# yang-0201/MAF-YOLO

Measured on AMD Instinct MI355X. Metric: images/sec MAF-YOLO-n 640x640 bs=32 infer (Model.forward + non_max_suppression), higher is better.
Workload: dtype f16

## Files before the change

maf-yolo_amd/csrc/conv1dw.hip:

```cpp
#include "maf_common.h"

namespace {

struct C1dArgs {
    const half_t* x; half_t* out;
    const unsigned char* par;
    int B, H, W, Cin, Cmid, S1, nMB, x_stride, x_coff, out_stride, out_coff;
    int tilesX, tilesY, nwg, rec;
};

typedef half_t half4v_t __attribute__((ext_vector_type(4)));

template <int K>
struct C1dCfg {
    static constexpr int P = K / 2, PARTS = K > 5 ? 2 : 1;
    static constexpr int RH = 16 + K - 1, RWC = (16 + K - 1 + 3) & ~3, NHP = RH * RWC, NPT = (NHP + 15) / 16;
    static constexpr int RWP = 24;
    static constexpr int PSB = ((RH * RWP * 2 - 8 + 255) / 256) * 256 + 8;
    static constexpr int PS = PSB / 2;
    static constexpr int NTOE = 8 * K * PARTS * 16;
};

template <int K>
__global__ __launch_bounds__(256) void conv1dw_kernel(const C1dArgs a) {
    typedef C1dCfg<K> Cf;
    constexpr int P = Cf::P, PARTS = Cf::PARTS, RWC = Cf::RWC, NHP = Cf::NHP, NPT = Cf::NPT, RWP = Cf::RWP, PS = Cf::PS;
    extern __shared__ __attribute__((aligned(16))) unsigned char smem_raw[];
    half_t* T1 = reinterpret_cast<half_t*>(smem_raw);
    unsigned char* rec = smem_raw + 32 * Cf::PSB;
    const int OFF_B1 = 2 * a.S1 * 1024, OFF_TOE = OFF_B1 + 128, OFF_BD = OFF_TOE + Cf::NTOE * 16;

    const int tid = threadIdx.x, wave = tid >> 6, lane = tid & 63, g = lane >> 4, p = lane & 15;
    const int lid = maf_xcd_contiguous_id(a.nwg);
    const int mb = lid % a.nMB;
    int tt = lid / a.nMB;
    const int tx = tt % a.tilesX; tt /= a.tilesX;
    const int ty = tt % a.tilesY;
    const int b = tt / a.tilesY;
    const int y0 = ty * 16, x0 = tx * 16;
    const half_t* xin = a.x + (size_t)b * a.H * a.W * a.x_stride + a.x_coff;

    {
        const unsigned char* src = a.par + (size_t)mb * a.rec;
        const int nvec = a.rec >> 4;
        for (int v0 = wave * 64; v0 < nvec; v0 += 256)
            if (v0 + lane < nvec)
                __builtin_amdgcn_global_load_lds((const void __attribute__((address_space(1)))*)(src + (size_t)(v0 + lane) * 16),
                                                 (void __attribute__((address_space(3)))*)(rec + v0 * 16), 16, 0, 0);
    }
    __syncthreads();

    {
        const bool interior = y0 - P >= 0 && x0 - P >= 0 && y0 - P + Cf::RH <= a.H && x0 - P + RWC <= a.W;
        const half8_t* w1l = reinterpret_cast<const half8_t*>(rec) + lane;
        const float b1v0 = reinterpret_cast<const float*>(rec + OFF_B1)[p], b1v1 = reinterpret_cast<const float*>(rec + OFF_B1)[16 + p];
        for (int t = wave; t < NPT; t += 4) {
            const int m = t * 16 + p;
            const int hrp = m / RWC, hcp = m - hrp * RWC;
            const int iy = min(max(y0 - P + hrp, 0), a.H - 1), ix = min(max(x0 - P + hcp, 0), a.W - 1);
            const half_t* px = xin + (size_t)(iy * a.W + ix) * a.x_stride;
            f32x4_t acc1[2] = {(f32x4_t)0.f, (f32x4_t)0.f};
            for (int ks0 = 0; ks0 < a.S1; ks0 += 4) {
                half8_t af[4];
#pragma unroll
                for (int u = 0; u < 4; ++u) {
                    int c = (ks0 + u) * 32 + g * 8;
                    c = c < a.Cin ? c : 0;
                    af[u] = *reinterpret_cast<const half8_t*>(px + c);
                }
#pragma unroll
                for (int u = 0; u < 4; ++u)
                    if (ks0 + u < a.S1) {
                        acc1[0] = __builtin_amdgcn_mfma_f32_16x16x32_f16(af[u], w1l[(0 * a.S1 + ks0 + u) * 64], acc1[0], 0, 0, 0);
                        acc1[1] = __builtin_amdgcn_mfma_f32_16x16x32_f16(af[u], w1l[(1 * a.S1 + ks0 + u) * 64], acc1[1], 0, 0, 0);
                    }
            }
            const int m0 = t * 16 + g * 4;
            const int hr = m0 / RWC, hc0 = m0 - hr * RWC;
            uint32_t mlo = 0xffffffffu, mhi = 0xffffffffu;
            if (!interior) {
                const int iy2 = y0 - P + hr, ixb = x0 - P + hc0;
                const bool rowok = (unsigned)iy2 < (unsigned)a.H;
                const uint32_t k0 = (rowok && (unsigned)(ixb + 0) < (unsigned)a.W) ? 0x0000ffffu : 0u, k1 = (rowok && (unsigned)(ixb + 1) < (unsigned)a.W) ? 0xffff0000u : 0u;
                const uint32_t k2 = (rowok && (unsigned)(ixb + 2) < (unsigned)a.W) ? 0x0000ffffu : 0u, k3 = (rowok && (unsigned)(ixb + 3) < (unsigned)a.W) ? 0xffff0000u : 0u;
                mlo = k0 | k1; mhi = k2 | k3;
            }
            half_t* dst = T1 + (size_t)p * PS + hr * RWP + hc0;
#pragma unroll
            for (int ct = 0; ct < 2; ++ct) {
                const float bv = ct ? b1v1 : b1v0;
                const half2_t h01 = {(half_t)maf_act<MAF_ACT_SILU>(acc1[ct][0] + bv), (half_t)maf_act<MAF_ACT_SILU>(acc1[ct][1] + bv)};
                const half2_t h23 = {(half_t)maf_act<MAF_ACT_SILU>(acc1[ct][2] + bv), (half_t)maf_act<MAF_ACT_SILU>(acc1[ct][3] + bv)};
                const u32x2_t w = {__builtin_bit_cast(uint32_t, h01) & mlo, __builtin_bit_cast(uint32_t, h23) & mhi};
                if (m0 < NHP) *reinterpret_cast<u32x2_t*>(dst + (size_t)(16 * ct) * PS) = w;
            }
        }
    }
    __syncthreads();

    const bool toe_active = (p >> 2) == g;
    const int q4 = wave * 4;
    int hi_off = 4;
    asm volatile("" : "+v"(hi_off));
    f32x4_t dacc[8];
#pragma unroll
    for (int s = 0; s < 8; ++s) dacc[s] = (f32x4_t)0.f;
    const half8_t* tl = reinterpret_cast<const half8_t*>(rec + OFF_TOE) + p;
    const half_t* t1l = T1 + (size_t)g * PS + p * RWP + q4;
    const half_t* t1h = t1l + hi_off;
#pragma unroll 1
    for (int ky = 0; ky < K; ++ky) {
#pragma unroll
        for (int part = 0; part < PARTS; ++part) {
#pragma unroll
            for (int s = 0; s < 8; ++s) {
                half8_t av = (half8_t)(half_t)0;
                if (toe_active) av = tl[((s * K + ky) * PARTS + part) * 16];
                const int o = s * 4 * PS + ky * RWP + part * 4;
                const half4v_t lo = *reinterpret_cast<const half4v_t*>(t1l + o), hi = *reinterpret_cast<const half4v_t*>(t1h + o);
                const half8_t bv = {lo[0], lo[1], lo[2], lo[3], hi[0], hi[1], hi[2], hi[3]};
                dacc[s] = __builtin_amdgcn_mfma_f32_16x16x32_f16(av, bv, dacc[s], 0, 0, 0);
            }
        }
    }
    const int c0 = mb * 32 + g * 8;
    if (c0 >= a.Cmid) return;
    const f32x4_t bd0 = reinterpret_cast<const f32x4_t*>(rec + OFF_BD)[g * 2], bd1 = reinterpret_cast<const f32x4_t*>(rec + OFF_BD)[g * 2 + 1];
    const float bs[8] = {bd0[0], bd0[1], bd0[2], bd0[3], bd1[0], bd1[1], bd1[2], bd1[3]};
    const int oy = y0 + p;
    if (oy >= a.H) return;
    half_t* orow = a.out + ((size_t)b * a.H + oy) * a.W * a.out_stride + a.out_coff + c0;
#pragma unroll
    for (int r = 0; r < 4; ++r) {
        const int ox = x0 + q4 + r;
        if (ox >= a.W) continue;
        half8_t o;
#pragma unroll
        for (int s = 0; s < 8; ++s) o[s] = (half_t)maf_act<MAF_ACT_SILU>(dacc[s][r] + bs[s]);
        *reinterpret_cast<half8_t*>(orow + (size_t)ox * a.out_stride) = o;
    }
}

template <int K>
int launch_k(const C1dArgs& a, hipStream_t s) {
    const size_t lds = (size_t)32 * C1dCfg<K>::PSB + (size_t)a.rec;
    MAF_REQUIRE(lds <= 160 * 1024, "conv1dw: tile + record do not fit LDS");
    static bool attr = false;
    if (!attr) {
        int rc = maf_check_hip(hipFuncSetAttribute(reinterpret_cast<const void*>(&conv1dw_kernel<K>), hipFuncAttributeMaxDynamicSharedMemorySize, 160 * 1024), "hipFuncSetAttribute(conv1dw)");
        if (rc) return rc;
        attr = true;
    }
    hipLaunchKernelGGL((conv1dw_kernel<K>), dim3(a.nwg), dim3(256), lds, s, a);
    return maf_check_hip(hipGetLastError(), "conv1dw launch");
}

}

extern "C" int64_t maf_conv1dw_record_bytes(int32_t k, int32_t Cin) {
    const int parts = k > 5 ? 2 : 1, s1 = (Cin + 31) / 32;
    return (int64_t)2 * s1 * 1024 + 128 + (int64_t)8 * k * parts * 16 * 16 + 128;
}

int maf_launch_conv1dw(const maf_op_t* op, hipStream_t s) {
    MAF_REQUIRE(op->dtype == MAF_F16, "conv1dw: fp16 only");
    const maf_src_t& sr = op->src[0];
    MAF_REQUIRE(op->nsrc == 1 && sr.mode == MAF_SRC_DIRECT && sr.ptr && op->out && op->w, "conv1dw: one direct source, w = block records");
    MAF_REQUIRE(op->Cin % 8 == 0 && op->Cout % 8 == 0 && op->Cin <= 512, "conv1dw: Cin, Cmid multiples of 8, Cin <= 512");
    MAF_REQUIRE(sr.stride % 8 == 0 && sr.coff % 8 == 0 && op->out_stride % 8 == 0 && op->out_coff % 8 == 0, "conv1dw: stride/offset alignment");
    MAF_REQUIRE(op->act == MAF_ACT_SILU, "conv1dw: SiLU after both stages (common.py:905-909)");
    C1dArgs a;
    a.x = static_cast<const half_t*>(sr.ptr); a.out = static_cast<half_t*>(op->out);
    a.par = static_cast<const unsigned char*>(op->w);
    a.B = op->B; a.H = op->H; a.W = op->W; a.Cin = op->Cin; a.Cmid = op->Cout; a.S1 = (op->Cin + 31) / 32; a.nMB = (op->Cout + 31) / 32;
    a.x_stride = sr.stride; a.x_coff = sr.coff; a.out_stride = op->out_stride; a.out_coff = op->out_coff;
    a.tilesX = maf_cdiv(a.W, 16); a.tilesY = maf_cdiv(a.H, 16);
    a.nwg = a.B * a.tilesX * a.tilesY * a.nMB;
    a.rec = (int)maf_conv1dw_record_bytes(op->ksize, op->Cin);
    switch (op->ksize) {
        case 3: return launch_k<3>(a, s);
        case 5: return launch_k<5>(a, s);
        case 7: return launch_k<7>(a, s);
        case 9: return launch_k<9>(a, s);
        default: maf_set_error("conv1dw: k must be 3, 5, 7 or 9"); return MAF_E_UNSUPPORTED;
    }
}
```

maf-yolo_amd/plan_report.py:

```python
from . import lib, pack

_ESIZE = {lib.F16: 2, lib.F32: 4}


def kernel_name(plan, idx):
    o = plan.ops[idx]
    T = "_Float16" if o.dtype == lib.F16 else "float"
    if o.kind in (lib.OP_CONV1X1, lib.OP_CONV3X3S2):
        if o.kind == lib.OP_CONV3X3S2:
            var = 3
        elif o.nsrc == 1 and o.src[0].mode == lib.SRC_POOL2:
            var = 2
        elif o.nsrc == 1 and o.src[0].mode == lib.SRC_DIRECT:
            var = 0
        else:
            var = 1
        outf32 = "true" if (o.out_f32 and o.dtype == lib.F16) else "false"
        if o.tile_k == lib.CONV_STREAM:
            return "conv1x1_stream_kernel<%d, %d, %d>" % (o.tile_p, o.tile_c, -(-o.Cin // 32))
        if o.tile_k == lib.CONV3_LDS:
            return "conv3s2_lds_kernel<%d, %d, 4, %d>" % (o.Cin, o.Cout, o.nc)
        if o.tile_k == lib.CONV3_WREG:
            return "conv3s2_wreg_kernel<%d, %d, %d, %d, %d, %d>" % ((o.Cin, o.Cout) + pack.conv3x3_wreg_shape(o.Cin, o.Cout) + (2 if o.tile_p == 2 else 3, o.nc))
        if o.tile_k == lib.CONV_STREAM_LDS:
            return "conv1x1_stream_lds_kernel<%d, %d, %s, %d, false>" % (o.tile_c, sum(-(-o.src[k].C // 32) for k in range(o.nsrc)), "true" if var == 1 else "false", 8 if o.tile_p == 2 else 4)
        return "conv_mfma_kernel<%s, %d, %d, %d, %s, %s, %s, %s>" % (T, o.tile_p, o.tile_c, var, outf32, "true" if o.tile_k == lib.CONV_SPLITK else "false", "true" if o.tile_k in (lib.CONV_LDS, lib.CONV_DMA) else "false",
                                                                     "true" if o.tile_k == lib.CONV_DMA else "false")
    if o.kind == lib.OP_DWCONV:
        if o.tile_p == lib.DW_MFMA:
            return "dwconv_mfma_kernel<%d, %d>" % (o.ksize, o.act)
        if o.tile_p == lib.DW_PAIRS:
            return "dwconv_p2_kernel<%d, %d, %d>" % (o.ksize, o.act, (o.Cout // o.Cin) if lib.dw_tile_k_split(o.tile_k)[2] else 0)
        if o.tile_p == lib.DW_DOT2:
            return "dwconv_dot2_kernel<%d, 8, %d, %d>" % (o.ksize, 2 if lib.dw_tile_k_split(o.tile_k)[0] % 2 == 0 else 1, o.act)
        return "dwconv_tile_kernel<%s, %d, %d>" % (T, o.ksize, o.act)
    if o.kind == lib.OP_BOTTLENECK:
        return "bottleneck_kernel<%d, %d, %d, %d, %d>" % (o.ksize, -(-o.Cin // 32), 2 if o.Cout <= 32 else 4, o.nc // 16, o.nsrc if o.nc else 0)
    if o.kind == lib.OP_CONV1DW:
        return "conv1dw_kernel<%d>" % o.ksize
    if o.kind == lib.OP_HEADTAIL:
        return "head_tail_kernel<%d, %d>" % (o.Cin, 2 if o.Cin <= 128 else 1)
    if o.kind == lib.OP_STEM2:
        return "stem2_kernel<%d, %d, %d>" % (o.ksize, o.Cout, o.nc)
    return {lib.OP_STEM: "stem_kernel", lib.OP_SPPF_POOL: "sppf_pool_lds_kernel", lib.OP_DECODE: "decode_kernel"}[o.kind]

def algorithmic_bytes(plan, idx):
    o = plan.ops[idx]
    es = plan.es
    px = plan.B * o.H * o.W
    if o.kind == lib.OP_STEM:
        ies = {lib.F16: 2, lib.F32: 4, lib.U8: 1}[o.in_dtype]
        return plan.B * 3 * o.Hin * o.Win * ies + px * o.Cout * es + 27 * o.Cout * 4
    if o.kind == lib.OP_STEM2:
        ies = {lib.F16: 2, lib.F32: 4, lib.U8: 1}[o.in_dtype]
        return plan.B * 3 * o.Hin * o.Win * ies + px * (o.nc or o.Cout) * es + (27 * o.ksize + 9 * o.ksize * o.Cout + o.Cout * o.nc) * es
    if o.kind == lib.OP_CONV1X1:
        rd = 0
        for i in range(o.nsrc):
            f = {lib.SRC_DIRECT: 1.0, lib.SRC_UP2: 0.25, lib.SRC_POOL2: 4.0}[o.src[i].mode]
            rd += px * f * o.src[i].C * es
        oes = 4 if o.out_f32 else es
        return int(rd) + px * o.Cout * oes + o.Cin * o.Cout * es
    if o.kind == lib.OP_CONV3X3S2:
        pooled = px * o.nc * es + o.Cin * o.nc * es if "pool1" in plan._ops[idx] else 0
        return (2 if "twin" in plan._ops[idx] else 1) * (plan.B * o.Hin * o.Win * o.Cin * es + px * o.Cout * es + 9 * o.Cin * o.Cout * es) + pooled
    if o.kind == lib.OP_DWCONV:
        return px * (o.Cin + o.Cout) * es + o.ksize * o.ksize * o.Cout * es
    if o.kind == lib.OP_CONV1DW:
        return px * (o.Cin + o.Cout) * es + (o.Cin * o.Cout + o.ksize * o.ksize * o.Cout) * es
    if o.kind == lib.OP_BOTTLENECK:
        mid = o.tile_k * 32
        wts = (o.Cin * mid + o.ksize * o.ksize * mid + mid * o.Cout) * es
        if o.nc:
            return px * (o.nsrc * o.Cin + o.nc) * es + wts + (o.nsrc + 1) * o.Cin * o.nc * es
        return px * (o.Cin + o.Cout) * es + wts
    if o.kind == lib.OP_SPPF_POOL:
        return 4 * px * o.src[0].C * es
    if o.kind == lib.OP_HEADTAIL:
        return px * (2 * o.Cin * es + (5 + plan.nc) * 4) + 2 * (o.Cin * o.Cin + 80 * o.Cin) * es
    if o.kind == lib.OP_DECODE:
        anchors = sum(t.H * t.W for t, c, _ in plan.head_bufs if c is not None)
        return plan.B * anchors * ((plan.nc + 4 * (plan.reg_max + 1)) * 4 + (5 + plan.nc) * 4)
    return 0

def flops(plan, idx):
    o = plan.ops[idx]
    px = plan.B * o.H * o.W
    if o.kind == lib.OP_STEM:
        return 2 * px * 27 * o.Cout
    if o.kind == lib.OP_STEM2:
        return 2 * (4 * px * 27 * o.ksize + px * 9 * o.ksize * o.Cout + px * o.Cout * o.nc)
    if o.kind == lib.OP_CONV1X1:
        return 2 * px * o.Cin * o.Cout
    if o.kind == lib.OP_CONV3X3S2:
        return (2 if "twin" in plan._ops[idx] else 1) * 2 * px * 9 * o.Cin * o.Cout + (2 * px * o.Cin * o.nc if "pool1" in plan._ops[idx] else 0)
    if o.kind == lib.OP_DWCONV:
        return 2 * px * o.ksize * o.ksize * o.Cout
    if o.kind == lib.OP_CONV1DW:
        return 2 * px * (o.Cin * o.Cout + o.ksize * o.ksize * o.Cout)
    if o.kind == lib.OP_BOTTLENECK:
        mid = plan._ops[idx]["mid"]
        return 2 * px * (o.Cin * mid + o.ksize * o.ksize * mid + mid * o.Cout + (o.nsrc + 1) * o.Cin * o.nc)
    if o.kind == lib.OP_HEADTAIL:
        return 2 * px * (2 * o.Cin * o.Cin + o.Cin * (plan.nc + 4 * (plan.reg_max + 1)))
    return 0
```

Before: 17620.

## Pipeline conv1dw across multiple mid blocks per workgroup with register-prefetched weights

Each conv1dw workgroup now processes several 32-channel mid blocks in a loop instead of one. Only the depthwise record is copied into LDS, and the 1x1 weights are held in registers and loaded from global memory. The kernel is specialised on S1 so input reads and depthwise LDS reads can be software-pipelined with explicit waits, and LDS is capped so two workgroups fit per CU. The intent is to cut launch and halo overhead, overlap loads with MFMA, and raise occupancy, at the cost of more template variants, higher register pressure and less grid parallelism when nb > 1.

```diff
diff --git a/maf-yolo_amd/csrc/conv1dw.hip b/maf-yolo_amd/csrc/conv1dw.hip
--- a/maf-yolo_amd/csrc/conv1dw.hip
+++ b/maf-yolo_amd/csrc/conv1dw.hip
@@ -1,4 +1,5 @@
 #include "maf_common.h"
+#include "lds_pipe.h"
 
 namespace {
 
@@ -7,152 +8,301 @@
     const unsigned char* par;
     int B, H, W, Cin, Cmid, S1, nMB, x_stride, x_coff, out_stride, out_coff;
     int tilesX, tilesY, nwg, rec;
+    int nb, ngrp;
 };
-
-typedef half_t half4v_t __attribute__((ext_vector_type(4)));
 
 template <int K>
 struct C1dCfg {
     static constexpr int P = K / 2, PARTS = K > 5 ? 2 : 1;
     static constexpr int RH = 16 + K - 1, RWC = (16 + K - 1 + 3) & ~3, NHP = RH * RWC, NPT = (NHP + 15) / 16;
+    static constexpr int MT = (NPT + 3) / 4;
     static constexpr int RWP = 24;
     static constexpr int PSB = ((RH * RWP * 2 - 8 + 255) / 256) * 256 + 8;
     static constexpr int PS = PSB / 2;
     static constexpr int NTOE = 8 * K * PARTS * 16;
+    static constexpr int OFF_TOE = 128, OFF_BD = OFF_TOE + NTOE * 16, REC_L = OFF_BD + 128;
+    static constexpr size_t LDS = (size_t)32 * PSB + REC_L;
+    static_assert(LDS <= 80 * 1024, "conv1dw: two workgroups per CU");
 };
 
-template <int K>
-__global__ __launch_bounds__(256) void conv1dw_kernel(const C1dArgs a) {
+#ifndef MAF_C1D_KO
+#define MAF_C1D_KO 0
+#endif
+constexpr int C1D_KO = MAF_C1D_KO;
+__device__ __forceinline__ float c1d_silu_a(float v) { return (C1D_KO & 2) ? v : maf_act<MAF_ACT_SILU>(v); }
+#ifdef MAF_C1D_TOE_AND
+constexpr bool C1D_TOE_AND = true;
+#else
+constexpr bool C1D_TOE_AND = false;
+#endif
+
+template <int OFF> __device__ __forceinline__ void c1d_read_b128_lanes(u32x4_t& d, uint32_t addr, uint64_t lanes) {
+    uint64_t keep;
+    asm volatile("s_and_saveexec_b64 %1, %3\n\tds_read_b128 %0, %2 offset:%4\n\ts_mov_b64 exec, %1" : "+v"(d), "=&s"(keep) : "v"(addr), "s"(lanes), "n"(OFF) : "scc");
+}
+
+template <int K, int S1T>
+__global__ __launch_bounds__(256, 2) void conv1dw_kernel(const C1dArgs a) {
     typedef C1dCfg<K> Cf;
-    constexpr int P = Cf::P, PARTS = Cf::PARTS, RWC = Cf::RWC, NHP = Cf::NHP, NPT = Cf::NPT, RWP = Cf::RWP, PS = Cf::PS;
+    constexpr int P = Cf::P, PARTS = Cf::PARTS, RWC = Cf::RWC, NHP = Cf::NHP, NPT = Cf::NPT, MT = Cf::MT, RWP = Cf::RWP, PS = Cf::PS;
     extern __shared__ __attribute__((aligned(16))) unsigned char smem_raw[];
     half_t* T1 = reinterpret_cast<half_t*>(smem_raw);
     unsigned char* rec = smem_raw + 32 * Cf::PSB;
-    const int OFF_B1 = 2 * a.S1 * 1024, OFF_TOE = OFF_B1 + 128, OFF_BD = OFF_TOE + Cf::NTOE * 16;
+    const int OFF_B1 = 2 * a.S1 * 1024;
 
     const int tid = threadIdx.x, wave = tid >> 6, lane = tid & 63, g = lane >> 4, p = lane & 15;
     const int lid = maf_xcd_contiguous_id(a.nwg);
-    const int mb = lid % a.nMB;
-    int tt = lid / a.nMB;
+    const int grp = lid % a.ngrp;
+    int tt = lid / a.ngrp;
     const int tx = tt % a.tilesX; tt /= a.tilesX;
     const int ty = tt % a.tilesY;
     const int b = tt / a.tilesY;
     const int y0 = ty * 16, x0 = tx * 16;
+    const int mb0 = grp * a.nb, mb1 = min(mb0 + a.nb, a.nMB);
     const half_t* xin = a.x + (size_t)b * a.H * a.W * a.x_stride + a.x_coff;
 
-    {
-        const unsigned char* src = a.par + (size_t)mb * a.rec;
-        const int nvec = a.rec >> 4;
+    auto dma_rec = [&](int mb) {
+        const unsigned char* src = a.par + (size_t)mb * a.rec + OFF_B1;
+        constexpr int nvec = Cf::REC_L >> 4;
         for (int v0 = wave * 64; v0 < nvec; v0 += 256)
             if (v0 + lane < nvec)
                 __builtin_amdgcn_global_load_lds((const void __attribute__((address_space(1)))*)(src + (size_t)(v0 + lane) * 16),
                                                  (void __attribute__((address_space(3)))*)(rec + v0 * 16), 16, 0, 0);
-    }
-    __syncthreads();
-
-    {
-        const bool interior = y0 - P >= 0 && x0 - P >= 0 && y0 - P + Cf::RH <= a.H && x0 - P + RWC <= a.W;
-        const half8_t* w1l = reinterpret_cast<const half8_t*>(rec) + lane;
-        const float b1v0 = reinterpret_cast<const float*>(rec + OFF_B1)[p], b1v1 = reinterpret_cast<const float*>(rec + OFF_B1)[16 + p];
-        for (int t = wave; t < NPT; t += 4) {
-            const int m = t * 16 + p;
-            const int hrp = m / RWC, hcp = m - hrp * RWC;
-            const int iy = min(max(y0 - P + hrp, 0), a.H - 1), ix = min(max(x0 - P + hcp, 0), a.W - 1);
-            const half_t* px = xin + (size_t)(iy * a.W + ix) * a.x_stride;
-            f32x4_t acc1[2] = {(f32x4_t)0.f, (f32x4_t)0.f};
-            for (int ks0 = 0; ks0 < a.S1; ks0 += 4) {
-                half8_t af[4];
-#pragma unroll
-                for (int u = 0; u < 4; ++u) {
-                    int c = (ks0 + u) * 32 + g * 8;
-                    c = c < a.Cin ? c : 0;
-                    af[u] = *reinterpret_cast<const half8_t*>(px + c);
-                }
-#pragma unroll
-                for (int u = 0; u < 4; ++u)
-                    if (ks0 + u < a.S1) {
-                        acc1[0] = __builtin_amdgcn_mfma_f32_16x16x32_f16(af[u], w1l[(0 * a.S1 + ks0 + u) * 64], acc1[0], 0, 0, 0);
-                        acc1[1] = __builtin_amdgcn_mfma_f32_16x16x32_f16(af[u], w1l[(1 * a.S1 + ks0 + u) * 64], acc1[1], 0, 0, 0);
-                    }
-            }
-            const int m0 = t * 16 + g * 4;
+    };
+
+    const bool interior = y0 - P >= 0 && x0 - P >= 0 && y0 - P + Cf::RH <= a.H && x0 - P + RWC <= a.W;
+    auto halo_mask = [&](int m0, uint32_t& mlo, uint32_t& mhi) {
+        mlo = mhi = 0xffffffffu;
+        if (!interior) {
             const int hr = m0 / RWC, hc0 = m0 - hr * RWC;
-            uint32_t mlo = 0xffffffffu, mhi = 0xffffffffu;
-            if (!interior) {
-                const int iy2 = y0 - P + hr, ixb = x0 - P + hc0;
-                const bool rowok = (unsigned)iy2 < (unsigned)a.H;
-                const uint32_t k0 = (rowok && (unsigned)(ixb + 0) < (unsigned)a.W) ? 0x0000ffffu : 0u, k1 = (rowok && (unsigned)(ixb + 1) < (unsigned)a.W) ? 0xffff0000u : 0u;
-                const uint32_t k2 = (rowok && (unsigned)(ixb + 2) < (unsigned)a.W) ? 0x0000ffffu : 0u, k3 = (rowok && (unsigned)(ixb + 3) < (unsigned)a.W) ? 0xffff0000u : 0u;
-                mlo = k0 | k1; mhi = k2 | k3;
-            }
-            half_t* dst = T1 + (size_t)p * PS + hr * RWP + hc0;
-#pragma unroll
-            for (int ct = 0; ct < 2; ++ct) {
-                const float bv = ct ? b1v1 : b1v0;
-                const half2_t h01 = {(half_t)maf_act<MAF_ACT_SILU>(acc1[ct][0] + bv), (half_t)maf_act<MAF_ACT_SILU>(acc1[ct][1] + bv)};
-                const half2_t h23 = {(half_t)maf_act<MAF_ACT_SILU>(acc1[ct][2] + bv), (half_t)maf_act<MAF_ACT_SILU>(acc1[ct][3] + bv)};
-                const u32x2_t w = {__builtin_bit_cast(uint32_t, h01) & mlo, __builtin_bit_cast(uint32_t, h23) & mhi};
-                if (m0 < NHP) *reinterpret_cast<u32x2_t*>(dst + (size_t)(16 * ct) * PS) = w;
-            }
-        }
-    }
-    __syncthreads();
-
-    const bool toe_active = (p >> 2) == g;
+            const int iy = y0 - P + hr, ixb = x0 - P + hc0;
+            const bool rowok = (unsigned)iy < (unsigned)a.H;
+            const uint32_t k0 = (rowok && (unsigned)(ixb + 0) < (unsigned)a.W) ? 0x0000ffffu : 0u, k1 = (rowok && (unsigned)(ixb + 1) < (unsigned)a.W) ? 0xffff0000u : 0u;
+            const uint32_t k2 = (rowok && (unsigned)(ixb + 2) < (unsigned)a.W) ? 0x0000ffffu : 0u, k3 = (rowok && (unsigned)(ixb + 3) < (unsigned)a.W) ? 0xffff0000u : 0u;
+            mlo = k0 | k1; mhi = k2 | k3;
+        }
+    };
+    auto halo_dst = [&](int m0) { const int hr = m0 / RWC, hc0 = m0 - hr * RWC; return m0 < NHP ? p * PS + hr * RWP + hc0 : -1; };
+    auto halo_xoff = [&](int m) {
+        const int hr = m / RWC, hc = m - hr * RWC;
+        const int iy = min(max(y0 - P + hr, 0), a.H - 1), ix = min(max(x0 - P + hc, 0), a.W - 1);
+        return (uint32_t)(iy * a.W + ix) * a.x_stride;
+    };
+
+    constexpr int S1 = S1T > 0 ? S1T : 1;
+    constexpr int XD = S1T == 6 ? (K == 7 ? 1 : 2) : S1T == 4 ? 1 : S1T == 3 ? 2 : 3;
+    static_assert(XD < MT, "read-ahead deeper than the wave's m-tiles");
+    constexpr int MTH = MT;
+    uint32_t xoff[MTH], tmlo[MTH], tmhi[MTH];
+    int tdst[MTH], cg[S1];
+    half8_t af[XD + 1][S1], w1f[2][S1];
+    float b1v0 = 0.f, b1v1 = 0.f;
+    if constexpr ((C1D_KO & 4) != 0) {
+#pragma unroll
+        for (int i = 0; i <= XD; ++i)
+#pragma unroll
+            for (int ks = 0; ks < S1; ++ks) af[i][ks] = (half8_t)(half_t)0;
+    }
+    auto load_x = [&](auto idx) {
+        constexpr int i = decltype(idx)::value;
+        if constexpr (i < MT && !(C1D_KO & 4)) {
+#pragma unroll
+            for (int ks = 0; ks < S1; ++ks) af[i % (XD + 1)][ks] = *reinterpret_cast<const half8_t*>(reinterpret_cast<const unsigned char*>(xin) + (uint32_t)(xoff[i] + cg[ks]));
+        }
+    };
+    auto load_x_head = [&]() { maf_static_for<XD>([&](auto idx) { load_x(idx); }); };
+    auto load_w = [&](int mb) {
+        const unsigned char* src = a.par + (size_t)mb * a.rec;
+#pragma unroll
+        for (int ct = 0; ct < 2; ++ct)
+#pragma unroll
+            for (int ks = 0; ks < S1; ++ks) w1f[ct][ks] = reinterpret_cast<const half8_t*>(src)[(ct * S1 + ks) * 64 + lane];
+        b1v0 = reinterpret_cast<const float*>(src + OFF_B1)[p]; b1v1 = reinterpret_cast<const float*>(src + OFF_B1)[16 + p];
+    };
+    auto set_cg = [&]() {
+        int g8 = g * 8;
+        asm volatile("" : "+v"(g8));
+#pragma unroll
+        for (int ks = 0; ks < S1; ++ks) cg[ks] = (ks * 32 + g8 < a.Cin ? ks * 32 + g8 : 0) * 2;
+    };
+    if constexpr (S1T > 0) {
+        set_cg();
+#pragma unroll
+        for (int i = 0; i < MT; ++i) {
+            xoff[i] = halo_xoff((wave + 4 * i) * 16 + p) * 2;
+            const int m0 = (wave + 4 * i) * 16 + g * 4;
+            halo_mask(m0, tmlo[i], tmhi[i]);
+            tdst[i] = halo_dst(m0);
+        }
+    }
+
+    const uint32_t toe_mask = (p >> 2) == g ? 0xffffffffu : 0u;
     const int q4 = wave * 4;
     int hi_off = 4;
     asm volatile("" : "+v"(hi_off));
-    f32x4_t dacc[8];
-#pragma unroll
-    for (int s = 0; s < 8; ++s) dacc[s] = (f32x4_t)0.f;
-    const half8_t* tl = reinterpret_cast<const half8_t*>(rec + OFF_TOE) + p;
-    const half_t* t1l = T1 + (size_t)g * PS + p * RWP + q4;
-    const half_t* t1h = t1l + hi_off;
-#pragma unroll 1
-    for (int ky = 0; ky < K; ++ky) {
-#pragma unroll
-        for (int part = 0; part < PARTS; ++part) {
-#pragma unroll
-            for (int s = 0; s < 8; ++s) {
-                half8_t av = (half8_t)(half_t)0;
-                if (toe_active) av = tl[((s * K + ky) * PARTS + part) * 16];
-                const int o = s * 4 * PS + ky * RWP + part * 4;
-                const half4v_t lo = *reinterpret_cast<const half4v_t*>(t1l + o), hi = *reinterpret_cast<const half4v_t*>(t1h + o);
-                const half8_t bv = {lo[0], lo[1], lo[2], lo[3], hi[0], hi[1], hi[2], hi[3]};
-                dacc[s] = __builtin_amdgcn_mfma_f32_16x16x32_f16(av, bv, dacc[s], 0, 0, 0);
+    const int oy = y0 + p;
+
+    dma_rec(mb0);
+    if constexpr (S1T > 0) { load_w(mb0); load_x_head(); }
+
+    for (int mb = mb0; mb < mb1; ++mb) {
+        if (mb > mb0) dma_rec(mb);
+        if constexpr ((C1D_KO & 16) != 0) {
+        } else if constexpr (S1T > 0) {
+            f32x4_t accn[2];
+            auto mma_tile = [&](auto idx) {
+                constexpr int i = decltype(idx)::value;
+                if constexpr (i < MT) {
+                    accn[0] = (f32x4_t)0.f; accn[1] = (f32x4_t)0.f;
+#pragma unroll
+                    for (int ks = 0; ks < S1; ++ks)
+#pragma unroll
+                        for (int ct = 0; ct < 2; ++ct) accn[ct] = __builtin_amdgcn_mfma_f32_16x16x32_f16(af[i % (XD + 1)][ks], w1f[ct][ks], accn[ct], 0, 0, 0);
+                }
+            };
+            mma_tile(std::integral_constant<int, 0>{});
+            maf_static_for<MT>([&](auto idx) {
+                constexpr int i = decltype(idx)::value;
+                load_x(std::integral_constant<int, i + XD>{});
+                f32x4_t acc1[2] = {accn[0], accn[1]};
+                mma_tile(std::integral_constant<int, i + 1>{});
+                __builtin_amdgcn_sched_barrier(0);
+                half_t* dst = T1 + tdst[i];
+#pragma unroll
+                for (int ct = 0; ct < 2; ++ct) {
+                    const float bv = ct ? b1v1 : b1v0;
+                    const half2_t h01 = {(half_t)c1d_silu_a(acc1[ct][0] + bv), (half_t)c1d_silu_a(acc1[ct][1] + bv)};
+                    const half2_t h23 = {(half_t)c1d_silu_a(acc1[ct][2] + bv), (half_t)c1d_silu_a(acc1[ct][3] + bv)};
+                    const u32x2_t w = {__builtin_bit_cast(uint32_t, h01) & tmlo[i], __builtin_bit_cast(uint32_t, h23) & tmhi[i]};
+                    if (tdst[i] >= 0) *reinterpret_cast<u32x2_t*>(dst + (size_t)(16 * ct) * PS) = w;
+                }
+            });
+        } else {
+            const unsigned char* src = a.par + (size_t)mb * a.rec;
+            const half8_t* w1l = reinterpret_cast<const half8_t*>(src) + lane;
+            const float bv0 = reinterpret_cast<const float*>(src + OFF_B1)[p], bv1 = reinterpret_cast<const float*>(src + OFF_B1)[16 + p];
+            for (int t = wave; t < NPT; t += 4) {
+                const half_t* px = xin + halo_xoff(t * 16 + p);
+                f32x4_t acc1[2] = {(f32x4_t)0.f, (f32x4_t)0.f};
+                for (int ks0 = 0; ks0 < a.S1; ks0 += 4) {
+                    half8_t xf[4], wf[2][4];
+#pragma unroll
+                    for (int u = 0; u < 4; ++u) {
+                        int c = (ks0 + u) * 32 + g * 8;
+                        c = c < a.Cin ? c : 0;
+                        xf[u] = *reinterpret_cast<const half8_t*>(px + c);
+                        const int ks = min(ks0 + u, a.S1 - 1);
+                        wf[0][u] = w1l[(0 * a.S1 + ks) * 64]; wf[1][u] = w1l[(1 * a.S1 + ks) * 64];
+                    }
+#pragma unroll
+                    for (int u = 0; u < 4; ++u)
+                        if (ks0 + u < a.S1) {
+                            acc1[0] = __builtin_amdgcn_mfma_f32_16x16x32_f16(xf[u], wf[0][u], acc1[0], 0, 0, 0);
+                            acc1[1] = __builtin_amdgcn_mfma_f32_16x16x32_f16(xf[u], wf[1][u], acc1[1], 0, 0, 0);
+                        }
+                }
+                const int m0 = t * 16 + g * 4;
+                uint32_t mlo, mhi;
+                halo_mask(m0, mlo, mhi);
+                const int doff = halo_dst(m0);
+                half_t* dst = T1 + doff;
+#pragma unroll
+                for (int ct = 0; ct < 2; ++ct) {
+                    const float bv = ct ? bv1 : bv0;
+                    const half2_t h01 = {(half_t)c1d_silu_a(acc1[ct][0] + bv), (half_t)c1d_silu_a(acc1[ct][1] + bv)};
+                    const half2_t h23 = {(half_t)c1d_silu_a(acc1[ct][2] + bv), (half_t)c1d_silu_a(acc1[ct][3] + bv)};
+                    const u32x2_t w = {__builtin_bit_cast(uint32_t, h01) & mlo, __builtin_bit_cast(uint32_t, h23) & mhi};
+                    if (doff >= 0) *reinterpret_cast<u32x2_t*>(dst + (size_t)(16 * ct) * PS) = w;
+                }
             }
         }
-    }
-    const int c0 = mb * 32 + g * 8;
-    if (c0 >= a.Cmid) return;
-    const f32x4_t bd0 = reinterpret_cast<const f32x4_t*>(rec + OFF_BD)[g * 2], bd1 = reinterpret_cast<const f32x4_t*>(rec + OFF_BD)[g * 2 + 1];
-    const float bs[8] = {bd0[0], bd0[1], bd0[2], bd0[3], bd1[0], bd1[1], bd1[2], bd1[3]};
-    const int oy = y0 + p;
-    if (oy >= a.H) return;
-    half_t* orow = a.out + ((size_t)b * a.H + oy) * a.W * a.out_stride + a.out_coff + c0;
-#pragma unroll
-    for (int r = 0; r < 4; ++r) {
-        const int ox = x0 + q4 + r;
-        if (ox >= a.W) continue;
-        half8_t o;
-#pragma unroll
-        for (int s = 0; s < 8; ++s) o[s] = (half_t)maf_act<MAF_ACT_SILU>(dacc[s][r] + bs[s]);
-        *reinterpret_cast<half8_t*>(orow + (size_t)ox * a.out_stride) = o;
-    }
+        lp_wait_vm<0>();
+        __syncthreads();
+        if constexpr (S1T > 0) {
+            if (mb + 1 < mb1) { set_cg(); load_w(mb + 1); load_x_head(); }
+        }
+
+        f32x4_t dacc[8];
+#pragma unroll
+        for (int s = 0; s < 8; ++s) dacc[s] = (f32x4_t)0.f;
+        const f32x4_t bd0 = reinterpret_cast<const f32x4_t*>(rec + Cf::OFF_BD)[g * 2], bd1 = reinterpret_cast<const f32x4_t*>(rec + Cf::OFF_BD)[g * 2 + 1];
+        const float bs[8] = {bd0[0], bd0[1], bd0[2], bd0[3], bd1[0], bd1[1], bd1[2], bd1[3]};
+        {
+            constexpr int NSTEP = K * PARTS * 8, BD = 3;
+            u32x4_t avr[BD + 1];
+            u32x2_t blo[BD + 1], bhi[BD + 1];
+            const half_t* t1l = T1 + (size_t)g * PS + p * RWP + q4;
+            const uint32_t a_toe = lp_lds_addr(rec + Cf::OFF_TOE + p * 16);
+            const uint32_t a_t1l = lp_lds_addr(t1l), a_t1h = lp_lds_addr(t1l + hi_off);
+            auto ld_step = [&](auto idx) {
+                constexpr int t = decltype(idx)::value;
+                if constexpr (t < NSTEP) {
+                    constexpr int s = t % 8, part = (t / 8) % PARTS, ky = t / (8 * PARTS);
+                    constexpr int ot = ((s * K + ky) * PARTS + part) * 256, o = (s * 4 * PS + ky * RWP + part * 4) * 2;
+                    static_assert(ot < 65536 && o < 65536, "ds offset field");
+                    if constexpr (C1D_TOE_AND) lp_ds_read_b128<ot>(avr[t % (BD + 1)], a_toe);
+                    else c1d_read_b128_lanes<ot>(avr[t % (BD + 1)], a_toe, 0xF0000F0000F0000Full);
+                    lp_ds_read_b64<o>(blo[t % (BD + 1)], a_t1l);
+                    lp_ds_read_b64<o>(bhi[t % (BD + 1)], a_t1h);
+                }
+            };
+#pragma unroll
+            for (int i = 0; i <= BD; ++i) avr[i] = (u32x4_t){0u, 0u, 0u, 0u};
+            lp_wait_lgkm<0>();
+            if constexpr (!(C1D_KO & 1)) {
+            maf_static_for<BD>([&](auto idx) { ld_step(idx); });
+            maf_static_for<NSTEP>([&](auto idx) {
+                constexpr int t = decltype(idx)::value, s = t % 8, sl = t % (BD + 1);
+                ld_step(std::integral_constant<int, t + BD>{});
+                constexpr int ahead = (NSTEP - 1 - t) < BD ? (NSTEP - 1 - t) : BD;
+                lp_wait_lgkm<3 * ahead>(avr[sl], blo[sl], bhi[sl]);
+                const u32x4_t bw = {blo[sl][0], blo[sl][1], bhi[sl][0], bhi[sl][1]};
+                const u32x4_t am = C1D_TOE_AND ? (avr[sl] & toe_mask) : avr[sl];
+                dacc[s] = __builtin_amdgcn_mfma_f32_16x16x32_f16(__builtin_bit_cast(half8_t, am), __builtin_bit_cast(half8_t, bw), dacc[s], 0, 0, 0);
+                __builtin_amdgcn_sched_barrier(0);
+            });
+            }
+        }
+        const int c0 = mb * 32 + g * 8;
+        if (c0 < a.Cmid && oy < a.H && !(C1D_KO & 8)) {
+            half_t* orow = a.out + ((size_t)b * a.H + oy) * a.W * a.out_stride + a.out_coff + c0;
+#pragma unroll
+            for (int r = 0; r < 4; ++r) {
+                const int ox = x0 + q4 + r;
+                if (ox >= a.W) continue;
+                half8_t o;
+#pragma unroll
+                for (int s = 0; s < 8; ++s) o[s] = (half_t)maf_act<MAF_ACT_SILU>(dacc[s][r] + bs[s]);
+                *reinterpret_cast<half8_t*>(orow + (size_t)ox * a.out_stride) = o;
+            }
+        }
+        if (mb + 1 < mb1) __syncthreads();
+    }
+}
+
+template <int K, int S1T>
+int launch_ks(const C1dArgs& a, hipStream_t s) {
+    constexpr size_t lds = C1dCfg<K>::LDS;
+    static bool attr = false;
+    if (!attr) {
+        int rc = maf_check_hip(hipFuncSetAttribute(reinterpret_cast<const void*>(&conv1dw_kernel<K, S1T>), hipFuncAttributeMaxDynamicSharedMemorySize, (int)lds), "hipFuncSetAttribute(conv1dw)");
+        if (rc) return rc;
+        attr = true;
+    }
+    hipLaunchKernelGGL((conv1dw_kernel<K, S1T>), dim3(a.nwg), dim3(256), lds, s, a);
+    return maf_check_hip(hipGetLastError(), "conv1dw launch");
 }
 
 template <int K>
 int launch_k(const C1dArgs& a, hipStream_t s) {
-    const size_t lds = (size_t)32 * C1dCfg<K>::PSB + (size_t)a.rec;
-    MAF_REQUIRE(lds <= 160 * 1024, "conv1dw: tile + record do not fit LDS");
-    static bool attr = false;
-    if (!attr) {
-        int rc = maf_check_hip(hipFuncSetAttribute(reinterpret_cast<const void*>(&conv1dw_kernel<K>), hipFuncAttributeMaxDynamicSharedMemorySize, 160 * 1024), "hipFuncSetAttribute(conv1dw)");
-        if (rc) return rc;
-        attr = true;
-    }
-    hipLaunchKernelGGL((conv1dw_kernel<K>), dim3(a.nwg), dim3(256), lds, s, a);
-    return maf_check_hip(hipGetLastError(), "conv1dw launch");
+    switch (a.S1) {
+        case 1: return launch_ks<K, 1>(a, s);
+        case 2: return launch_ks<K, 2>(a, s);
+        case 3: return launch_ks<K, 3>(a, s);
+        case 4: return launch_ks<K, 4>(a, s);
+        case 6: return launch_ks<K, 6>(a, s);
+        default: return launch_ks<K, 0>(a, s);
+    }
 }
 
 }
@@ -160,6 +310,17 @@
 extern "C" int64_t maf_conv1dw_record_bytes(int32_t k, int32_t Cin) {
     const int parts = k > 5 ? 2 : 1, s1 = (Cin + 31) / 32;
     return (int64_t)2 * s1 * 1024 + 128 + (int64_t)8 * k * parts * 16 * 16 + 128;
+}
+
+static int conv1dw_blocks_per_wg(int tiles, int nMB) {
+    int best = 1;
+    long bestcost = (long)((tiles * nMB + 511) / 512);
+    for (int nb = 2; nb <= 4 && nb <= nMB; ++nb) {
+        const int nwg = tiles * ((nMB + nb - 1) / nb);
+        const long cost = (long)((nwg + 511) / 512) * nb;
+        if (nwg >= 512 && cost <= bestcost) { best = nb; bestcost = cost; }
+    }
+    return best;
 }
 
 int maf_launch_conv1dw(const maf_op_t* op, hipStream_t s) {
@@ -169,13 +330,17 @@
     MAF_REQUIRE(op->Cin % 8 == 0 && op->Cout % 8 == 0 && op->Cin <= 512, "conv1dw: Cin, Cmid multiples of 8, Cin <= 512");
     MAF_REQUIRE(sr.stride % 8 == 0 && sr.coff % 8 == 0 && op->out_stride % 8 == 0 && op->out_coff % 8 == 0, "conv1dw: stride/offset alignment");
     MAF_REQUIRE(op->act == MAF_ACT_SILU, "conv1dw: SiLU after both stages (common.py:905-909)");
+    MAF_REQUIRE(op->tile_k >= 0 && op->tile_k <= 64, "conv1dw: tile_k = mid blocks per workgroup (0: the built-in rule)");
     C1dArgs a;
     a.x = static_cast<const half_t*>(sr.ptr); a.out = static_cast<half_t*>(op->out);
     a.par = static_cast<const unsigned char*>(op->w);
     a.B = op->B; a.H = op->H; a.W = op->W; a.Cin = op->Cin; a.Cmid = op->Cout; a.S1 = (op->Cin + 31) / 32; a.nMB = (op->Cout + 31) / 32;
     a.x_stride = sr.stride; a.x_coff = sr.coff; a.out_stride = op->out_stride; a.out_coff = op->out_coff;
     a.tilesX = maf_cdiv(a.W, 16); a.tilesY = maf_cdiv(a.H, 16);
-    a.nwg = a.B * a.tilesX * a.tilesY * a.nMB;
+    const int tiles = a.B * a.tilesX * a.tilesY;
+    a.nb = op->tile_k > 0 ? (op->tile_k < a.nMB ? op->tile_k : a.nMB) : conv1dw_blocks_per_wg(tiles, a.nMB);
+    a.ngrp = (a.nMB + a.nb - 1) / a.nb;
+    a.nwg = tiles * a.ngrp;
     a.rec = (int)maf_conv1dw_record_bytes(op->ksize, op->Cin);
     switch (op->ksize) {
         case 3: return launch_k<3>(a, s);
diff --git a/maf-yolo_amd/plan_report.py b/maf-yolo_amd/plan_report.py
--- a/maf-yolo_amd/plan_report.py
+++ b/maf-yolo_amd/plan_report.py
@@ -37,7 +37,8 @@
     if o.kind == lib.OP_BOTTLENECK:
         return "bottleneck_kernel<%d, %d, %d, %d, %d>" % (o.ksize, -(-o.Cin // 32), 2 if o.Cout <= 32 else 4, o.nc // 16, o.nsrc if o.nc else 0)
     if o.kind == lib.OP_CONV1DW:
-        return "conv1dw_kernel<%d>" % o.ksize
+        s1 = -(-o.Cin // 32)
+        return "conv1dw_kernel<%d, %d>" % (o.ksize, s1 if s1 in (1, 2, 3, 4, 6) else 0)
     if o.kind == lib.OP_HEADTAIL:
         return "head_tail_kernel<%d, %d>" % (o.Cin, 2 if o.Cin <= 128 else 1)
     if o.kind == lib.OP_STEM2:
```

Result: slower. 15470 (-12.2%).
